# twndus/YelpRecommendation

Hardware: AMD Instinct MI355X
Metric: BPR triplets/sec @ dim64 (higher is better)
Workload: dtype f32; 1 GPU; BPR-MF dim=64 train step (gather+score+loss+grad+dense Adam), synthetic Yelp2018 shape; users=31668, items=38048, interactions=1566260, train_triplets_per_epoch=920629, batch_per_gpu=524288, global_batch=524288, optimizer=adam(dense), parallelism=single

## Files before the change

include/yelprec_engine.h:

```cpp
#ifndef YELPREC_ENGINE_H
#define YELPREC_ENGINE_H

#include <stdint.h>

#ifdef __cplusplus
extern "C" {
#endif

#define YR_ENGINE_VERSION 31

#define YR_ERR_UNSUPPORTED (-1)
#define YR_ERR_BADARG      (-2)

#define YR_FLAG_BAD_USER 1
#define YR_FLAG_BAD_ITEM 2

#define YR_PULL_USER_PHASE 1
#define YR_PULL_ITEM_PHASE 2

#define YR_OPT_ADAM  0
#define YR_OPT_ADAMW 1

#define YR_LOSS_PARTIALS 2048
#define YR_COUNT_SLOTS 64
#define YR_COUNT_WORDS 2048

int yr_engine_version(void);

const char *yr_engine_arch(void);

int yr_mf_score(const float *U, const float *I,
                const int64_t *user, const int64_t *item,
// ... 31 lines not shown
int yr_bpr_mf_pull_step(const float *U_old, float *U_new, float *I,
                        float *mU, float *vU, float *mI, float *vI, float *gradI_out,
                        const int64_t *user, const int64_t *pos, const int64_t *neg,
                        int64_t B, int D, int64_t num_users, int64_t num_items, float inv_batch,
                        double lr, double step_size, double bc2_sqrt,
                        double beta1, double beta2, double eps, double weight_decay, int mode,
                        int deterministic, void *workspace, int64_t workspace_bytes,
                        float *loss_partials, float *loss_out, double *loss_accum,
                        int32_t *err_flag, void *stream);

int yr_bpr_mf_pull_index(const int64_t *user, const int64_t *pos, const int64_t *neg, int64_t B, int D,
                         int64_t num_users, int64_t num_items,
                         void *workspace, int64_t workspace_bytes, int32_t *err_flag, void *stream);
int yr_bpr_mf_pull_apply(const float *U_old, float *U_new, float *I,
                         float *mU, float *vU, float *mI, float *vI, float *gradI_out,
                         int64_t B, int D, int64_t num_users, int64_t num_items, float inv_batch,
                         double lr, double step_size, double bc2_sqrt,
                         double beta1, double beta2, double eps, double weight_decay, int mode,
                         int deterministic, void *workspace, int64_t workspace_bytes,
                         float *loss_partials, float *loss_out, double *loss_accum,
                         int phases, int64_t item_row_begin, int64_t item_row_end,
                         void *stream);
int yr_bpr_mf_pull_item_buckets(int64_t num_items, int D);
int yr_bpr_mf_pull_apply_ordered(const float *U_old, float *U_new, float *I,
                         float *mU, float *vU, float *mI, float *vI, float *gradI_out,
                         int64_t B, int D, int64_t num_users, int64_t num_items, float inv_batch,
                         double lr, double step_size, double bc2_sqrt,
                         double beta1, double beta2, double eps, double weight_decay, int mode,
                         int deterministic, void *workspace, int64_t workspace_bytes,
                         float *loss_partials, float *loss_out, double *loss_accum,
                         int phases, int64_t item_row_begin, int64_t item_row_end,
                         const int32_t *item_bucket_order, void *stream);

#define YR_NGCF_MAX_LAYERS 8
int yr_ngcf_score_fwd(const float *const *layers, int n_layers, const int64_t *user, const int64_t *pos,
                      const int64_t *neg, int64_t B, int D, int64_t num_users, int64_t num_items,
                      float *out_pos, float *out_neg, int32_t *err_flag, void *stream);
int yr_ngcf_score_bwd(const float *const *layers, float *const *dlayers, int n_layers, const int64_t *user,
                      const int64_t *pos, const int64_t *neg, const float *gpos, const float *gneg,
                      int64_t B, int D, int64_t num_users, int64_t num_items, int32_t *err_flag, void *stream);
int yr_spmm_csr(const int32_t *rowptr, const int32_t *col, const float *val,
                const float *X, float *Y, int64_t n, int D, int accumulate,
                const int32_t *heavy_rows, int64_t n_heavy, int heavy_threshold, void *stream);
int yr_spmm_csr_sliced(const int32_t *rowptr, const int32_t *col, const float *val,
                       const float *X, float *Y, int64_t n, int D, int accumulate,
                       const int32_t *row_order, void *stream);
// ... 217 lines not shown
```

yelprecommendation_amd/_lib.py:

```python
from __future__ import annotations

import ctypes as C
import os

_HERE = os.path.dirname(os.path.abspath(__file__))
LIB_PATH = os.environ.get("YR_ENGINE_LIB") or os.path.join(_HERE, "libyelprec_engine.so")
ENGINE_VERSION = 31

_p = C.c_void_p
_i64 = C.c_int64
_int = C.c_int
_f = C.c_float
_d = C.c_double

SIGNATURES = {
    "yr_engine_version": [],
    "yr_engine_arch": [],
    "yr_mf_score": [_p, _p, _p, _p, _i64, _int, _i64, _i64, _p, _p, _p],
    "yr_mf_score_backward": [_p, _p, _p, _p, _p, _i64, _int, _i64, _i64, _p, _p, _p, _p],
    "yr_bpr_mf_fwd_bwd": [_p, _p, _p, _p, _p, _i64, _int, _i64, _i64, _f, _p, _p, _p, _p, _p],
    "yr_bpr_mf_scatter_step": [_p, _p, _p, _p, _p, _p, _p, _p, _p, _p, _p, _p, _i64, _int, _i64, _i64, _f,
                               _d, _d, _d, _d, _d, _d, _d, _int, _p, _p, _p, _p, _p],
    "yr_adam_dense_dual": [_p, _p, _p, _p, _i64, _p, _p, _p, _p, _i64, _int, _p, _p,
                           _d, _d, _d, _d, _d, _d, _d, _int, _p, _f, _p, _p, _p],
    "yr_bpr_mf_pull_workspace_bytes": [_i64, _i64, _i64, _int],
    "yr_bpr_mf_pull_step": [_p, _p, _p, _p, _p, _p, _p, _p, _p, _p, _p, _i64, _int, _i64, _i64, _f,
                            _d, _d, _d, _d, _d, _d, _d, _int, _int, _p, _i64, _p, _p, _p, _p, _p],
    "yr_spmm_csr": [_p, _p, _p, _p, _p, _i64, _int, _int, _p, _i64, _int, _p],
    "yr_spmm_csr_sliced": [_p, _p, _p, _p, _p, _i64, _int, _int, _p, _p],
    "yr_ngcf_score_fwd": [_p, _int, _p, _p, _p, _i64, _int, _i64, _i64, _p, _p, _p, _p],
# ... 20 lines not shown
    "yr_cdae_train_lists": [_p, _p, _p, _p, _p, _i64, _i64, _i64, _int, C.c_uint64, C.c_uint64, _d, _p, _p, _p, _p, _p,
                            _p, _p, _p],
    "yr_cdae_train_lists_batched": [_p, _p, _p, _p, _p, _i64, _i64, _i64, _int, _p, _p, _i64, _d, _p, _p, _p, _p, _p,
                                    _p, _p, _p],
    "yr_cdae_loss_finalize_batched": [_p, _int, _p, _i64, _i64, _p, _p, _p, _p],
    "yr_cdae_loss_finalize": [_p, _i64, _p, _p, _p, _p],
    "yr_cdae_sampled_decode_splits": [_i64],
    "yr_cdae_sampled_decode": [_p, _p, _p, _p, _p, _p, _i64, _i64, _int, _int, _p, _p, _p, _p, _p, _p],
    "yr_cdae_hidden_init": [_p, _p, _p, _p, _i64, _int, _i64, _p, _p],
    "yr_dropout": [_p, _p, _d, _i64, _p, _p],
    "yr_sigmoid": [_p, _i64, _p],
    "yr_dropout_seeded": [_p, C.c_uint64, _d, _i64, _p, _p],
    "yr_sigmoid_bwd": [_p, _p, _p, _i64, _p],
    "yr_colsum": [_p, _i64, _i64, _p, _int, _p],
    "yr_row_scatter_add": [_p, _p, _i64, _int, _i64, _p, _p],
    "yr_nsbce_fwd": [_p, _p, _p, _i64, _p, _p, _p],
    "yr_nsbce_bwd": [_p, _p, _p, _p, _p, _i64, _p, _p],
    "yr_bpr_mf_pull_index": [_p, _p, _p, _i64, _int, _i64, _i64, _p, _i64, _p, _p],
    "yr_bpr_mf_pull_apply": [_p, _p, _p, _p, _p, _p, _p, _p, _i64, _int, _i64, _i64, _f,
                             _d, _d, _d, _d, _d, _d, _d, _int, _int, _p, _i64, _p, _p, _p, _int, _i64, _i64, _p],
    "yr_bpr_mf_pull_apply_ordered": [_p, _p, _p, _p, _p, _p, _p, _p, _i64, _int, _i64, _i64, _f,
                             _d, _d, _d, _d, _d, _d, _d, _int, _int, _p, _i64, _p, _p, _p, _int, _i64, _i64, _p, _p],
    "yr_bpr_mf_pull_item_buckets": [_i64, _int],
    "yr_loss_finalize": [_p, _f, _p, _p, _p],
    "yr_mf_scores_gemm": [_p, _p, _p, _i64, _int, _i64, _i64, _p, _i64, _p, _p],
    "yr_mf_eval_topk_planes_bytes": [_i64, _int],
    "yr_mf_eval_topk_workspace_bytes": [_i64, _i64, _int, _int, _int],
    "yr_mf_eval_topk": [_p, _p, _p, _i64, _int, _i64, _i64, _p, _p, _f, _int, _p, _p, _i64, _int, _p, _p, _p],
    "yr_mf_eval_topk_bias": [_p, _p, _p, _p, _i64, _int, _i64, _i64, _p, _p, _f, _int, _p, _p, _i64, _int, _p, _p, _p],
    "yr_topk_masked": [_p, _i64, _i64, _i64, _p, _p, _p, _f, _int, _p, _p],
    "yr_rank_metrics_workspace_bytes": [_i64],
    "yr_rank_metrics": [_p, _i64, _int, _p, _p, _p, _p, _p, _p],
    "yr_bpr_loss_fwd": [_p, _p, _i64, _p, _p],
    "yr_bpr_loss_bwd": [_p, _p, _p, _f, _i64, _p, _p, _p],
    "yr_adam_dense": [_p, _p, _p, _p, _i64, _d, _d, _d, _d, _d, _d, _d, _int, _int, _p],
    "yr_adam_dense_flat": [_p, _p, _p, _p, _p, _p, _p, _p, _p, _p, _int, _d, _d, _d, _d, _d, _d, _d, _int, _p],
    "yr_csr_rows_to_dense": [_p, _p, _p, _i64, _i64, _i64, _int, _p, _p, _p],
    "yr_negative_mask": [_p, _i64, _i64, _int, C.c_uint64, _p, _p, _p],
    "yr_sgd_dense": [_p, _p, _i64, _d, _d, _int, _p],
    "yr_cdae_sparse_part_columns": [_i64],
    "yr_cdae_compact_rows": [_p, _i64, _i64, C.c_uint64, _d, _p, _p, _p, _p],
    "yr_cdae_sparse_encode": [_p, _p, _p, _p, _p, _p, _p, _i64, _i64, _int, _i64, _int, _p, _p, _p],
    "yr_cdae_sparse_dwh": [_p, _p, _p, _p, _i64, _i64, _int, _p, _p, _p, C.c_int32, _p, _p, _p],
    "yr_cdae_sparse_encode_t": [_p, _p, _p, _p, _p, _p, _p, _i64, _i64, _int, _i64, _int, _p, _p, _p],
    "yr_cdae_sparse_dwh_t": [_p, _p, _p, _p, _i64, _i64, _int, _p, _p, _p],
    "yr_cdae_hidden_bwd_dwh_t": [_p, _p, _p, _p, _p, _int, _int, _p, _p, _i64, _i64, _int, _i64, _p, _p, _p, _p, _p, _p,
# ... 67 lines not shown
```

yelprecommendation_amd/csrc/bpr_pull.hip:

```cpp
#include "adam.h"
#include "common.h"

namespace yr {

constexpr int kPartThreads = 1024;
#ifndef YR_ITEM_CAP
#define YR_ITEM_CAP 1024
#endif
constexpr int kCap = YR_ITEM_CAP;
constexpr int kUserCap = 768;
constexpr int kTileGroup = 256;
constexpr int kOccShift = 26;
constexpr int kOccMask = (1 << kOccShift) - 1;
constexpr int kMaxBuckets = 16383;
constexpr int kMaxOwnerGrid = 4096;
#ifndef YR_HEAVY_ROW
#define YR_HEAVY_ROW 96
#endif
constexpr int kHeavyRow = YR_HEAVY_ROW;
#ifndef YR_SPLIT_MIN
#define YR_SPLIT_MIN 2048
#endif
constexpr int kSplitMin = YR_SPLIT_MIN;
#ifndef YR_SPLIT_AVG_MIN
#define YR_SPLIT_AVG_MIN 2.5
#endif
#ifndef YR_SPLIT_AVG_TARGET
#define YR_SPLIT_AVG_TARGET 1.25
#endif
#ifndef YR_SPLIT_TARGET
#define YR_SPLIT_TARGET 1024
#endif
constexpr int kSplitTarget = YR_SPLIT_TARGET;
constexpr int kMaxParts = 64;
constexpr int kMaxTasks = 512;
constexpr int kMaxSlots = 1024;
constexpr int kBuildLanes = 4;
#ifndef YR_DEAL
#define YR_DEAL 1
#endif
#ifndef YR_DEAL_MIN
#define YR_DEAL_MIN 256
#endif
constexpr int kDealMin = YR_DEAL_MIN;
#ifndef YR_OWNER_WAVES
#define YR_OWNER_WAVES 8
#endif

struct PullAdam {
  AdamScalars c;
  int decoupled;
};

__device__ __forceinline__ float4 ld4o(const float* base, uint32_t off) {
  return *reinterpret_cast<const float4*>(reinterpret_cast<const char*>(base) + (uint32_t)(off * 4u));
}

template <int D>
struct PullGeom {
// ... 8 lines not shown
constexpr int kMinTiles = YR_MIN_TILES;
constexpr int kNarrowRows = kWavesPerBlock;
constexpr int kNarrowShift = 2;
#ifndef YR_NARROW_BELOW
#define YR_NARROW_BELOW 768
#endif
constexpr int kNarrowBelow = YR_NARROW_BELOW;

inline int bucket_shift(int D) { return D == 16 ? 6 : D == 32 ? 5 : D == 64 ? 4 : 3; }

template <int PT>
__global__ __launch_bounds__(kPartThreads) void tile_partition_kernel(
    const int64_t* __restrict__ user, const int64_t* __restrict__ pos, const int64_t* __restrict__ neg, int64_t B,
    int64_t nU, int64_t nI, int shiftU, int shiftI, int nbU, int nbI, int32_t* __restrict__ offU,
    int32_t* __restrict__ offI,
    int4* __restrict__ rec, int2* __restrict__ occ, int32_t* __restrict__ err_flag, int stage_off,
    int32_t* __restrict__ split_counters) {
  extern __shared__ int32_t s_cnt[];
  __shared__ int s_wave[kPartThreads / kWave];
  int4* s_stage = reinterpret_cast<int4*>(s_cnt + stage_off);
  constexpr int TILE = kPartThreads * PT;
  const int side = blockIdx.y, tile = blockIdx.x, tid = threadIdx.x;
  if (side == 0 && tile == 0) {
    if (tid < 2) split_counters[tid] = 0;
    for (int i = tid; i < nbI; i += kPartThreads) split_counters[4 + i] = 1;
  }
  const int nb = side ? nbI : nbU;
  const int shift = side ? shiftI : shiftU;
  const int rmask = (1 << shift) - 1;

  int32_t u[PT], p[PT], n[PT];
  int bad = 0;
#pragma unroll
  for (int k = 0; k < PT; ++k) {
    const int64_t b = (int64_t)tile * TILE + (int64_t)k * kPartThreads + tid;
    u[k] = -1; p[k] = 0; n[k] = 0;
    if (b < B) {
      const int64_t uu = user[b], pp = pos[b], nn = neg[b];
      int f = 0;
      if ((uint64_t)uu >= (uint64_t)nU) f |= YR_FLAG_BAD_USER;
      if ((uint64_t)pp >= (uint64_t)nI || (uint64_t)nn >= (uint64_t)nI) f |= YR_FLAG_BAD_ITEM;
      if (f) bad |= f;
      else { u[k] = (int32_t)uu; p[k] = (int32_t)pp; n[k] = (int32_t)nn; }
    }
  }
  for (int i = tid; i <= nb; i += kPartThreads) s_cnt[i] = 0;
  __syncthreads();
// ... 79 lines not shown
  const float* other;
  float* m;
  float* v;
  float* grad_out;
  const int32_t* off;
  const void* recs;
  float* coeff;
  float* loss_partials;
  float* loss_out;
  double* loss_accum;
  int finalize;
  int nb, T, tile_stride;
  int rows;
  int bucket_begin, bucket_end;
  const int32_t* order;
  int heavy_t;
  float inv_batch;
  PullAdam adam;
  char* split;
  float* scratch;
  const int32_t* b_off;
  int helper_blocks, build_blocks, b_nb;
  int b_split_min, b_split_target;
};

__host__ __device__ __forceinline__ size_t split_per(int nbI) { return ((size_t)nbI * 4 + 15) & ~(size_t)15; }
__device__ __forceinline__ int32_t* split_counters(char* b) { return (int32_t*)b; }
__device__ __forceinline__ int32_t* split_parts(char* b) { return (int32_t*)(b + 16); }
__device__ __forceinline__ int32_t* split_slot(char* b, int nbI) { return (int32_t*)(b + 16 + split_per(nbI)); }
__device__ __forceinline__ int32_t* split_arrive(char* b, int nbI) { return (int32_t*)(b + 16 + 2 * split_per(nbI)); }
__device__ __forceinline__ int4* split_tasks(char* b, int nbI) { return (int4*)(b + 16 + 3 * split_per(nbI)); }

__device__ __forceinline__ void build_splits(const OwnerArgs& a, int builder) {
  const int k = (builder * kBlock + (int)threadIdx.x) / kBuildLanes, j = threadIdx.x % kBuildLanes;
  int total = 0;
  if (k < a.b_nb) {
    int t = j;
    const int64_t pitch = a.b_nb + 1;
    for (; t + 3 * kBuildLanes < a.T; t += 4 * kBuildLanes) {
      const int32_t* o0 = a.b_off + (int64_t)t * pitch + k;
      const int32_t* o1 = o0 + kBuildLanes * pitch;
      const int32_t* o2 = o1 + kBuildLanes * pitch;
      const int32_t* o3 = o2 + kBuildLanes * pitch;
      const int a0 = o0[0], b0 = o0[1], a1 = o1[0], b1 = o1[1], a2 = o2[0], b2 = o2[1], a3 = o3[0], b3 = o3[1];
      total += ((b0 - a0) + (b1 - a1)) + ((b2 - a2) + (b3 - a3));
    }
    for (; t < a.T; t += kBuildLanes) {
      const int32_t* orow = a.b_off + (int64_t)t * (a.b_nb + 1) + k;
      total += orow[1] - orow[0];
    }
  }
#pragma unroll
  for (int m = 1; m < kBuildLanes; m <<= 1) total += __shfl_xor(total, m, kWave);
  if (k >= a.b_nb || j != 0) return;
  int parts = 1;
  if (total >= a.b_split_min) {
    parts = (total + a.b_split_target - 1) / a.b_split_target;
    parts = min(parts, min(kMaxParts, a.T));
  }
  int slot = 0;
  if (parts > 1) {
    slot = atomicAdd(split_counters(a.split) + 1, parts);
    const int first = atomicAdd(split_counters(a.split), parts - 1);
    const bool fits = slot + parts <= kMaxSlots && first + parts - 1 <= kMaxTasks;
    for (int q = 1; q < parts; ++q)
      if (first + q - 1 < kMaxTasks) split_tasks(a.split, a.b_nb)[first + q - 1] = make_int4(fits ? k : -1, q, 0, 0);
    if (!fits) parts = 1;
  }
  split_parts(a.split)[k] = parts;
  split_slot(a.split, a.b_nb)[k] = slot;
  split_arrive(a.split, a.b_nb)[k] = 0;
}

template <int LPR>
__device__ __forceinline__ void cross_group_sum(float4& a) {
#pragma unroll
  for (int m = LPR; m < kWave; m <<= 1) {
    a.x += __shfl_xor(a.x, m, kWave);
    a.y += __shfl_xor(a.y, m, kWave);
    a.z += __shfl_xor(a.z, m, kWave);
    a.w += __shfl_xor(a.w, m, kWave);
  }
}

__device__ __forceinline__ int wave_inclusive_scan(int x, int lane) {
#pragma unroll
  for (int d = 1; d < kWave; d <<= 1) {
    const int t = __shfl_up(x, d, kWave);
    if (lane >= d) x += t;
  }
  return x;
// ... 104 lines not shown
        part = fmaf(ownj.z, d.z, part);
        part = fmaf(ownj.w, d.w, part);
        const float x = group_sum_dpp<LPR>(part);
        float sp, sg;
        bpr_terms(x, sp, sg);
        const float gg = valid[q] ? -sg * a.inv_batch : 0.0f;
        cur.x = fmaf(gg, d.x, cur.x); cur.y = fmaf(gg, d.y, cur.y);
        cur.z = fmaf(gg, d.z, cur.z); cur.w = fmaf(gg, d.w, cur.w);
        if (valid[q] && l == 0) {
          a.coeff[ic[q]] = gg;
          loss += sp;
        }
      } else {
        const float gg = valid[q] ? __int_as_float(ib[q]) : 0.0f;
        cur.x = fmaf(gg, r0[q].x, cur.x); cur.y = fmaf(gg, r0[q].y, cur.y);
        cur.z = fmaf(gg, r0[q].z, cur.z); cur.w = fmaf(gg, r0[q].w, cur.w);
      }
    }
  }
  if (!HEAVY) {
    const int slot = LOOKUP ? (int)s_slotof[max(cur_row, 0)] : cur_row;
    sums.book(cur_row >= 0, slot - row_base, cur, grp);
  }
}

template <int D, bool USER, bool FUSE_ADAM, bool DET, int RPWX = 0>
__global__ __launch_bounds__(kBlock, YR_OWNER_WAVES) void owner_pass_kernel(OwnerArgs a) {
  using G = PullGeom<D>;
  constexpr int LPR = G::LPR, GPW = G::GPW;
  constexpr int RPW = RPWX ? RPWX : GPW;
  static_assert(RPW <= GPW, "a wave finishes at most one row per lane group");
  constexpr int R = kWavesPerBlock * RPW;
  constexpr int DEAL_BAR = kDealMin * (kWavesPerBlock * GPW) * (kWavesPerBlock * GPW) / 256;
  constexpr bool DEAL = RPWX == 0 && YR_DEAL && DEAL_BAR <= (USER ? kUserCap : kCap);
  constexpr bool TAG_SLOT = DEAL && !USER, LOOKUP = DEAL && USER;
  constexpr int CAP = USER ? kUserCap : kCap;
  constexpr int PT = CAP / kBlock;
  __shared__ int s_pre[kTileGroup + 1];
  __shared__ int s_base[kTileGroup];
  __shared__ int s_cnt[kWave];
  __shared__ int s_start[kWave];
  __shared__ int s_light[kWave + 1];
  __shared__ unsigned char s_slotof[DEAL ? kWave : 1];
  __shared__ unsigned char s_rowof[DEAL ? kWave : 1];
  __shared__ int s_x[CAP];
  __shared__ int s_y[CAP];
// ... 6 lines not shown
  __shared__ int s_n;
  const int tid = threadIdx.x, lane = tid & (kWave - 1), wave = tid / kWave;
  const int grp = lane / LPR, l = lane % LPR;
  const bool finisher = grp < RPW;
  const int row_l = wave * RPW + (finisher ? grp : 0);
  float loss = 0.0f;
  __shared__ int s_last;
  if (USER && (int)blockIdx.x < a.build_blocks) {
    build_splits(a, blockIdx.x);
    return;
  }
  const int hb = USER ? a.build_blocks : a.helper_blocks;
  const bool helper = !USER && (int)blockIdx.x < hb;
  const int owners = (int)gridDim.x - hb;
#ifdef YR_STAMPS
  bool first_bucket = true;
  int walk_iters = 0, heavy_iters = 0;
#endif
  YR_STAMP(0);

  for (int ks = helper ? (int)blockIdx.x : a.bucket_begin + (int)blockIdx.x - hb;
       helper ? ks == (int)blockIdx.x : ks < a.bucket_end; ks += owners) {
    int k, part = 0, parts = 1;
    const bool pools_hold = USER || !a.split || (split_counters(a.split)[0] <= kMaxTasks &&
                                                 split_counters(a.split)[1] <= kMaxSlots);
    if (helper) {
      if (!pools_hold || ks >= split_counters(a.split)[0]) break;
      const int4 task = split_tasks(a.split, a.nb)[ks];
      k = __builtin_amdgcn_readfirstlane(task.x);
      part = __builtin_amdgcn_readfirstlane(task.y);
      if (k < a.bucket_begin || k >= a.bucket_end) break;
    } else {
      k = __builtin_amdgcn_readfirstlane(a.order ? a.order[ks] : ks);
    }
    if (!USER && a.split && pools_hold) parts = __builtin_amdgcn_readfirstlane(split_parts(a.split)[k]);
    const int t_begin = __builtin_amdgcn_readfirstlane(a.T * part / parts);
    const int t_end = __builtin_amdgcn_readfirstlane(a.T * (part + 1) / parts);
    int row_t = row_l;
    int row_f = k * R + row_t;
    bool valid_f = finisher && row_f < a.rows;
    uint32_t o_f = (uint32_t)(row_f * D + 4 * l);
    bool bound = false;
    if (USER && finisher) s_own[row_l * LPR + l] = valid_f ? ld4o(a.own_old, o_f) : zero4();
    YR_STAMP(1);
    RowSums<LPR, GPW> sums;
    sums.clear();

    for (int tg0 = t_begin; tg0 < t_end; tg0 += kTileGroup) {
      const int nt = min(kTileGroup, t_end - tg0);
      int len = 0;
      if (tid < nt) {
        const int32_t* orow = a.off + (int64_t)(tg0 + tid) * (a.nb + 1) + k;
        const int o0 = orow[0], o1 = orow[1];
        len = o1 - o0;
        s_base[tid] = (tg0 + tid) * a.tile_stride + o0;
      }
      int inc = 0, before = 0;
      if (nt > kWave) {
        inc = wave_inclusive_scan(len, lane);
        if (lane == kWave - 1) s_scan[wave] = inc;
        __syncthreads();
        for (int w = 0; w < wave; ++w) before += s_scan[w];
      } else if (wave == 0) {
// ... 30 lines not shown
        }
        if (tid < kWave) s_cnt[tid] = 0;
        if (DET && tid == 0) s_n = 0;
        __syncthreads();
        int key[PT];
        int n_rec = cend - c0;
        if (DET && windowed) {
          constexpr int W = USER ? CAP : CAP / 2;
          const int tile_ids = USER ? a.tile_stride : a.tile_stride >> 1;
          const int seg = s_pre[wt + 1] - s_pre[wt];
          const uint32_t rbase = (uint32_t)s_base[wt];
          const uint32_t id_lo = (uint32_t)(tg0 + wt) * (uint32_t)tile_ids + (uint32_t)sub * (uint32_t)W;
          for (int sidx = tid; sidx < seg; sidx += kBlock) {
            if (USER) {
              const int4 r = static_cast<const int4*>(a.recs)[rbase + sidx];
              if ((uint32_t)r.z - id_lo < (uint32_t)W) {
                const int slot = atomicAdd(&s_n, 1);
                s_x[slot] = r.x; s_y[slot] = r.y; s_z[slot] = r.z;
                s_idx[slot] = (unsigned short)r.w;
              }
            } else {
              const int2 oc = static_cast<const int2*>(a.recs)[rbase + sidx];
              const uint32_t b = (uint32_t)(oc.y & 0x7fffffff);
              if (b - id_lo < (uint32_t)W) {
                const float g = a.coeff[b];
                const int slot = atomicAdd(&s_n, 1);
                s_x[slot] = oc.x & kOccMask;
                s_y[slot] = __float_as_int(oc.y < 0 ? -g : g);
                s_z[slot] = oc.y;
                s_idx[slot] = (unsigned short)((uint32_t)oc.x >> kOccShift);
              }
            }
          }
          __syncthreads();
          n_rec = s_n;
#pragma unroll
          for (int q = 0; q < PT; ++q) {
            const int c = tid + q * kBlock;
            key[q] = -1;
            if (c < n_rec) {
              const int local = s_idx[c];
              key[q] = local | (atomicAdd(&s_cnt[local], 1) << 8);
            }
          }
          ++sub;
          if (sub * W >= tile_ids) { sub = 0; cend = s_pre[wt + 1]; }
          else cend = c0;
// ... 13 lines not shown
            if (s_pre[mid] <= j) tlo = mid; else thi = mid;
          }
          addr[q] = j < cend ? (uint32_t)(s_base[tlo] + (j - s_pre[tlo])) : 0u;
        }
        if (USER) {
          int4 r[PT];
#pragma unroll
          for (int q = 0; q < PT; ++q)
            r[q] = *reinterpret_cast<const int4*>(static_cast<const char*>(a.recs) + (uint32_t)(addr[q] * 16u));
#pragma unroll
          for (int q = 0; q < PT; ++q)
            if (key[q] >= 0) {
              const int c = tid + q * kBlock;
              s_x[c] = r[q].x; s_y[c] = r[q].y; s_z[c] = r[q].z;
              key[q] = r[q].w | (atomicAdd(&s_cnt[r[q].w], 1) << 8);
            }
        } else {
          int2 oc[PT];
          float g[PT];
#pragma unroll
          for (int q = 0; q < PT; ++q)
            oc[q] = *reinterpret_cast<const int2*>(static_cast<const char*>(a.recs) + (uint32_t)(addr[q] * 8u));
#pragma unroll
          for (int q = 0; q < PT; ++q) {
            const uint32_t b = key[q] >= 0 ? (uint32_t)(oc[q].y & 0x7fffffff) : 0u;
            g[q] = *reinterpret_cast<const float*>(reinterpret_cast<const char*>(a.coeff) + (uint32_t)(b * 4u));
          }
#pragma unroll
          for (int q = 0; q < PT; ++q)
            if (key[q] >= 0) {
              const int c = tid + q * kBlock;
              const int local = (int)((uint32_t)oc[q].x >> kOccShift);
              s_x[c] = oc[q].x & kOccMask;
              s_y[c] = __float_as_int(oc[q].y < 0 ? -g[q] : g[q]);
              if (DET) s_z[c] = oc[q].y;
              key[q] = local | (atomicAdd(&s_cnt[local], 1) << 8);
            }
        }
        }
        __syncthreads();
        if (wave == 0) {
          if (DEAL && !bound) {
            if (n_rec >= DEAL_BAR) {
              deal_rows<R, RPW>(s_cnt, s_slotof, s_rowof, lane, a.heavy_t);
            } else {
              s_slotof[lane] = (unsigned char)lane;
              s_rowof[lane] = (unsigned char)lane;
            }
            __builtin_amdgcn_fence(__ATOMIC_ACQ_REL, "wavefront");
            __builtin_amdgcn_wave_barrier();
          }
          const int row = DEAL ? (int)s_rowof[lane] : lane;
          const int c = s_cnt[row];
          const bool heavy = c > a.heavy_t;
          const int cl = heavy ? 0 : c, ch = heavy ? c : 0;
          const int il = wave_inclusive_scan(cl, lane), ih = wave_inclusive_scan(ch, lane);
          const int total_light = __shfl(il, kWave - 1, kWave);
          s_light[lane] = il - cl;
          if (lane == kWave - 1) s_light[kWave] = il;
          s_start[row] = heavy ? total_light + ih - ch : il - cl;
        }
        bound = true;
        __syncthreads();
#pragma unroll
        for (int q = 0; q < PT; ++q)
          if (key[q] >= 0) {
            const int row = key[q] & 255;
            const int tag = TAG_SLOT ? (int)s_slotof[row] : row;
            s_idx[s_start[row] + (key[q] >> 8)] = (unsigned short)((tid + q * kBlock) | (tag << kTagShift));
          }
        __syncthreads();
        if (DET) {
          int at[PT];
          unsigned short ent[PT];
#pragma unroll
          for (int q = 0; q < PT; ++q) {
            const int pos = tid + q * kBlock;
            at[q] = -1;
            if (pos < n_rec) {
              ent[q] = s_idx[pos];
              const int r = TAG_SLOT ? (int)s_rowof[ent[q] >> kTagShift] : ent[q] >> kTagShift;
              const uint32_t mine = (uint32_t)s_z[ent[q] & ((1 << kTagShift) - 1)];
              const int lo = s_start[r], cnt = s_cnt[r];
              int before = 0;
              for (int j = lo; j < lo + cnt; ++j)
                before += (uint32_t)s_z[s_idx[j] & ((1 << kTagShift) - 1)] < mine ? 1 : 0;
// ... 28 lines not shown
#endif
            cross_group_sum<LPR>(t);
            if (grp == 0) s_heavy[wave][l] = t;
            __syncthreads();
            if (finisher && row_l == (DEAL ? (int)s_slotof[r] : r)) {
#pragma unroll
              for (int w = 0; w < kWavesPerBlock; ++w) {
                const float4 h = s_heavy[w][l];
                sums.total.x += h.x; sums.total.y += h.y; sums.total.z += h.z; sums.total.w += h.w;
              }
            }
            __syncthreads();
          }
        }
        __syncthreads();
      }
    }

    YR_STAMP(3);
    float4 acc = sums.finish(grp);
    if (DEAL) {
      if (bound) row_t = s_rowof[row_l];
      row_f = k * R + row_t;
      valid_f = row_f < a.rows;
      int t2 = tid;
      asm volatile("" : "+v"(t2));
      o_f = (uint32_t)(row_f * D + 4 * (t2 % LPR));
    }
    if (!USER && parts > 1) {
      float* sbase = a.scratch;
      asm volatile("" : "+s"(sbase));
      float* slots = sbase + (int64_t)split_slot(a.split, a.nb)[k] * (R * D);
      if (finisher) st4(slots + (int64_t)part * (R * D) + row_t * D + 4 * l, acc);
      __threadfence();
      __syncthreads();
      if (tid == 0) {
        s_last = atomicAdd(split_arrive(a.split, a.nb) + k, 1) == parts - 1;
        if (s_last) split_arrive(a.split, a.nb)[k] = 0;
      }
      __syncthreads();
      const bool last = s_last != 0;
      __syncthreads();
      if (!last) continue;
      __threadfence();
      acc = zero4();
      if (finisher) {
        for (int q = 0; q < parts; ++q) {
          const float4 t = ld4(slots + (int64_t)q * (R * D) + row_t * D + 4 * l);
          acc.x += t.x; acc.y += t.y; acc.z += t.z; acc.w += t.w;
        }
      }
    }
    if (valid_f) {
      if (FUSE_ADAM) {
        float4 own = USER ? s_own[row_t * LPR + l] : ld4o(a.own_old, o_f);
        float4 M = ld4o(a.m, o_f), V = ld4o(a.v, o_f);
        adam_element(own.x, acc.x, M.x, V.x, a.adam.c, a.adam.decoupled);
        adam_element(own.y, acc.y, M.y, V.y, a.adam.c, a.adam.decoupled);
        adam_element(own.z, acc.z, M.z, V.z, a.adam.c, a.adam.decoupled);
        adam_element(own.w, acc.w, M.w, V.w, a.adam.c, a.adam.decoupled);
        st4(a.own_new + o_f, own);
        st4(a.m + o_f, M);
        st4(a.v + o_f, V);
      } else {
        st4(a.grad_out + o_f, acc);
      }
    }
    YR_STAMP(4);
    if (USER) __syncthreads();
    YR_STAMP(5);
#ifdef YR_STAMPS
// ... 24 lines not shown
    }
  }
}

__global__ __launch_bounds__(kBlock) void pull_loss_finalize_kernel(const float* __restrict__ partials, float scale,
                                                                    float* __restrict__ loss_out,
                                                                    double* __restrict__ loss_accum) {
  __shared__ float s_red[kWavesPerBlock];
  float s = 0.0f;
  for (int i = threadIdx.x; i < YR_LOSS_PARTIALS; i += kBlock) s += partials[i];
  const float total = block_sum(s, s_red);
  if (threadIdx.x == 0) {
    const float v = total * scale;
    if (loss_out) loss_out[0] = v;
    if (loss_accum) loss_accum[0] += (double)v;
  }
}

inline size_t align16(size_t x) { return (x + 15) & ~(size_t)15; }
struct PullPlan {
  int pt, tile, T, shiftU, shiftI, narrow_users, nbU, nbI;
  size_t o_offU, o_offI, o_rec, o_occ, o_coeff, o_split, o_scratch, bytes;
};
inline size_t split_bytes(int nbI) { return 16 + (size_t)3 * align16((size_t)nbI * 4) + (size_t)kMaxTasks * sizeof(int4); }

inline int tile_pt(int64_t B) {
  int pt = 4;
  while (pt > 1 && (B + (int64_t)kPartThreads * pt - 1) / ((int64_t)kPartThreads * pt) < kMinTiles) pt >>= 1;
  return pt;
}

inline PullPlan make_plan(int64_t B, int64_t nU, int64_t nI, int D, bool upper_bound) {
  PullPlan p;
  p.shiftI = bucket_shift(D);
  const int R = 1 << p.shiftI;
  p.narrow_users = (nU + R - 1) / R < kNarrowBelow && R > kNarrowRows;
  p.shiftU = p.narrow_users ? kNarrowShift : p.shiftI;
  p.nbU = (int)((nU + (1 << p.shiftU) - 1) >> p.shiftU);
  p.nbI = (int)((nI + (1 << p.shiftI) - 1) >> p.shiftI);
  p.pt = tile_pt(B);
  p.tile = kPartThreads * p.pt;
  p.T = (int)((B + p.tile - 1) / p.tile);
  const int64_t T = upper_bound ? ((B + 4095) / 4096 > 2 * kMinTiles ? (B + 4095) / 4096 : 2 * kMinTiles) : p.T;
  const int64_t slots = upper_bound ? B + 4096 : (int64_t)p.T * p.tile;
  size_t o = 0;
  p.o_offU = o; o += align16((size_t)T * (p.nbU + 1) * 4);
  p.o_offI = o; o += align16((size_t)T * (p.nbI + 1) * 4);
  p.o_rec = o; o += align16((size_t)slots * sizeof(int4));
  p.o_occ = o; o += align16((size_t)slots * 2 * sizeof(int2));
  p.o_coeff = o; o += align16((size_t)(B > 0 ? B : 1) * 4);
  p.o_split = o; o += align16(split_bytes(p.nbI));
  p.o_scratch = o; o += (size_t)kMaxSlots * 1024 * 4;
  p.bytes = o;
  return p;
}

}

using namespace yr;

static int pull_check_common(int64_t B, int D, int64_t num_users, int64_t num_items, const void* workspace,
                             int64_t workspace_bytes) {
  if (B < 0 || num_users <= 0 || num_items <= 0 || B > 0x3fffffff) return YR_ERR_BADARG;
  if (D != 16 && D != 32 && D != 64 && D != 128) return YR_ERR_UNSUPPORTED;
  const PullPlan pl = make_plan(0, num_users, num_items, D, false);
  if (pl.nbU > kMaxBuckets || pl.nbI > kMaxBuckets) return YR_ERR_UNSUPPORTED;
  if (num_users > kOccMask) return YR_ERR_UNSUPPORTED;
  if (!workspace || (reinterpret_cast<uintptr_t>(workspace) & 15u) != 0) return YR_ERR_BADARG;
  if ((int64_t)make_plan(B, num_users, num_items, D, false).bytes > workspace_bytes) return YR_ERR_BADARG;
  return 0;
}

#ifdef YR_STAMPS
extern "C" int yr_debug_read_stamps(long long* host, int n) {
  return (int)hipMemcpyFromSymbol(host, HIP_SYMBOL(g_stamps), sizeof(long long) * n);
}
extern "C" int yr_debug_read_walk_iters(int* host, int n) {
// ... 47 lines not shown
  return launch_status();
}

template <int D>
static int pull_apply_impl(const float* U_old, float* U_new, float* I, float* mU, float* vU, float* mI, float* vI,
                           float* gradI_out, int64_t B, int64_t nU, int64_t nI, float inv_batch, const PullAdam& adam,
                           int deterministic, void* workspace, float* loss_partials, float* loss_out,
                           double* loss_accum, int phases, int64_t item_begin, int64_t item_end,
                           const int32_t* item_order, hipStream_t s) {
  const PullPlan p = make_plan(B, nU, nI, D, false);
  char* w = static_cast<char*>(workspace);
  const bool want_loss = loss_out || loss_accum;
  if (phases & YR_PULL_USER_PHASE) {
    OwnerArgs ua{};
    ua.own_old = U_old; ua.own_new = U_new; ua.other = I; ua.m = mU; ua.v = vU; ua.grad_out = nullptr;
    ua.off = (const int32_t*)(w + p.o_offU); ua.recs = w + p.o_rec; ua.coeff = (float*)(w + p.o_coeff);
    ua.loss_partials = loss_partials;
    ua.nb = p.nbU; ua.T = p.T; ua.tile_stride = p.tile; ua.rows = (int)nU;
    ua.bucket_begin = 0; ua.bucket_end = p.nbU;
    ua.order = nullptr;
    ua.heavy_t = kHeavyRow; ua.inv_batch = inv_batch; ua.adam = adam;
    ua.build_blocks = (p.nbI * kBuildLanes + kBlock - 1) / kBlock;
    ua.b_off = (const int32_t*)(w + p.o_offI); ua.b_nb = p.nbI;
    {
      const double avg = 2.0 * (double)B / (double)p.nbI;
      const int by_avg_min = (int)(YR_SPLIT_AVG_MIN * avg), by_avg_target = (int)(YR_SPLIT_AVG_TARGET * avg);
      ua.b_split_min = by_avg_min > kSplitMin ? by_avg_min : kSplitMin;
      ua.b_split_target = by_avg_target > kSplitTarget ? by_avg_target : kSplitTarget;
    }
    ua.split = w + p.o_split;
    const int gu = (p.nbU < YR_LOSS_PARTIALS ? p.nbU : YR_LOSS_PARTIALS) + ua.build_blocks;
    if (p.narrow_users && deterministic)
      hipLaunchKernelGGL((owner_pass_kernel<D, true, true, true, 1>), dim3(gu), dim3(kBlock), 0, s, ua);
    else if (p.narrow_users)
      hipLaunchKernelGGL((owner_pass_kernel<D, true, true, false, 1>), dim3(gu), dim3(kBlock), 0, s, ua);
    else if (deterministic)
      hipLaunchKernelGGL((owner_pass_kernel<D, true, true, true>), dim3(gu), dim3(kBlock), 0, s, ua);
    else
      hipLaunchKernelGGL((owner_pass_kernel<D, true, true, false>), dim3(gu), dim3(kBlock), 0, s, ua);
  }
  const bool items = (phases & YR_PULL_ITEM_PHASE) && item_end > item_begin;
  if (items) {
    OwnerArgs ia{};
    ia.own_old = I; ia.own_new = I; ia.other = U_old; ia.m = mI; ia.v = vI; ia.grad_out = gradI_out;
    ia.off = (const int32_t*)(w + p.o_offI); ia.recs = w + p.o_occ; ia.coeff = (float*)(w + p.o_coeff);
    ia.loss_partials = loss_partials; ia.loss_out = loss_out; ia.loss_accum = loss_accum;
    ia.finalize = want_loss ? 1 : 0;
    ia.nb = p.nbI; ia.T = p.T; ia.tile_stride = 2 * p.tile; ia.rows = (int)nI;
    ia.bucket_begin = (int)(item_begin >> p.shiftI);
    ia.bucket_end = (int)((item_end + (1 << p.shiftI) - 1) >> p.shiftI);
    ia.order = (item_order && ia.bucket_begin == 0 && ia.bucket_end == p.nbI) ? item_order : nullptr;
    ia.heavy_t = kHeavyRow; ia.inv_batch = inv_batch; ia.adam = adam;
    ia.helper_blocks = kMaxTasks;
    ia.split = w + p.o_split;
    ia.scratch = (float*)(w + p.o_scratch);
    int gi = ia.bucket_end - ia.bucket_begin;
    if (gi > kMaxOwnerGrid) gi = kMaxOwnerGrid;
    gi += kMaxTasks;
    if (gradI_out && deterministic)
      hipLaunchKernelGGL((owner_pass_kernel<D, false, false, true>), dim3(gi), dim3(kBlock), 0, s, ia);
    else if (gradI_out)
      hipLaunchKernelGGL((owner_pass_kernel<D, false, false, false>), dim3(gi), dim3(kBlock), 0, s, ia);
    else if (deterministic)
      hipLaunchKernelGGL((owner_pass_kernel<D, false, true, true>), dim3(gi), dim3(kBlock), 0, s, ia);
    else
      hipLaunchKernelGGL((owner_pass_kernel<D, false, true, false>), dim3(gi), dim3(kBlock), 0, s, ia);
  } else if (want_loss) {
    hipLaunchKernelGGL(pull_loss_finalize_kernel, dim3(1), dim3(kBlock), 0, s, loss_partials, inv_batch, loss_out,
                       loss_accum);
  }
  return launch_status();
}

extern "C" int yr_bpr_mf_pull_item_buckets(int64_t num_items, int D) {
  if (num_items <= 0 || (D != 16 && D != 32 && D != 64 && D != 128)) return YR_ERR_BADARG;
  const int sh = bucket_shift(D);
  return (int)((num_items + (1 << sh) - 1) >> sh);
}

extern "C" int yr_bpr_mf_pull_apply_ordered(const float* U_old, float* U_new, float* I, float* mU, float* vU,
                                            float* mI, float* vI, float* gradI_out, int64_t B, int D,
                                            int64_t num_users, int64_t num_items, float inv_batch, double lr,
                                            double step_size, double bc2_sqrt, double beta1, double beta2, double eps,
                                            double weight_decay, int mode, int deterministic, void* workspace,
                                            int64_t workspace_bytes, float* loss_partials, float* loss_out,
                                            double* loss_accum, int phases, int64_t item_row_begin,
                                            int64_t item_row_end, const int32_t* item_bucket_order, void* stream) {
  int rc = pull_check_common(B, D, num_users, num_items, workspace, workspace_bytes);
  if (rc) return rc;
  if (!(phases & (YR_PULL_USER_PHASE | YR_PULL_ITEM_PHASE))) return YR_ERR_BADARG;
  if (item_row_begin < 0 || item_row_end > num_items || item_row_begin > item_row_end) return YR_ERR_BADARG;
  const int R = 1 << bucket_shift(D);
  if (item_row_begin % R != 0 || (item_row_end % R != 0 && item_row_end != num_items)) return YR_ERR_BADARG;
  if (!U_old || !U_new || U_old == U_new || !I || !mU || !vU || !loss_partials) return YR_ERR_BADARG;
  if (!gradI_out && (!mI || !vI)) return YR_ERR_BADARG;
  if (mode != YR_OPT_ADAM && mode != YR_OPT_ADAMW) return YR_ERR_UNSUPPORTED;
  const PullAdam c = {adam_scalars(lr, step_size, bc2_sqrt, beta1, beta2, eps, weight_decay), mode == YR_OPT_ADAMW};
  hipStream_t s = (hipStream_t)stream;
#define YR_APPLY_CASE(DD)                                                                                       \
  case DD:                                                                                                      \
// ... 45 lines not shown
```

yelprecommendation_amd/engine.py:

```python
from __future__ import annotations

import torch

from . import _lib
from ._lib import EngineError, check

LOSS_PARTIALS = 2048
FLAG_BAD_USER, FLAG_BAD_ITEM = 1, 2
OPT_ADAM, OPT_ADAMW = 0, 1
PULL_USER_PHASE, PULL_ITEM_PHASE = 1, 2
SUPPORTED_WIDTHS = (16, 32, 64, 128)
WIDE_WIDTHS = (256, 512, 1024)
MF_WIDTHS = SUPPORTED_WIDTHS + WIDE_WIDTHS


_raw_stream = getattr(torch._C, "_cuda_getCurrentRawStream", None)


def _stream() -> int:
    if _raw_stream is not None:
        return _raw_stream(torch.cuda.current_device())
    return torch.cuda.current_stream().cuda_stream


# ... 87 lines not shown
PULL_MAX_BUCKETS = 16383
PULL_MAX_USERS = (1 << 26) - 1


def pull_bucket_rows(d):
    return 1024 // int(d)


def pull_supported(num_users, num_items, d):
    if d not in SUPPORTED_WIDTHS:
        return False
    r = pull_bucket_rows(d)
    ru = 4 if (-(-num_users // r) < 768 and r > 4) else r
    return (-(-num_users // ru) <= PULL_MAX_BUCKETS and -(-num_items // r) <= PULL_MAX_BUCKETS
            and num_users <= PULL_MAX_USERS)


def bpr_mf_pull_workspace(max_batch, num_users, num_items, d, device):
    lib = _lib.load()
    n = lib.yr_bpr_mf_pull_workspace_bytes(int(max_batch), int(num_users), int(num_items), int(d))
    if n < 0:
        check(int(n), "yr_bpr_mf_pull_workspace_bytes")
    return torch.empty(int(n), dtype=torch.uint8, device=device)


def bpr_mf_pull_step(U_old, U_new, I, mU, vU, mI, vI, user, pos, neg, step, lr, loss_partials, workspace,
                     beta1=0.9, beta2=0.999, eps=1e-8, weight_decay=0.0, decoupled=False, inv_batch=None,
                     gradI_out=None, err_flag=None, loss_out=None, loss_accum=None, deterministic=False):
    lib = _lib.load()
    nu, ni, d = _table_dims(U_old, I)
    B = user.numel()
    if pos.numel() != B or neg.numel() != B:
        raise EngineError("user/pos/neg index tensors differ in length")
    if U_new.shape != U_old.shape or U_new.data_ptr() == U_old.data_ptr():
        raise EngineError("U_new must be a distinct buffer of U_old's shape")
    if loss_partials.numel() != LOSS_PARTIALS:
        raise EngineError(f"loss_partials must hold {LOSS_PARTIALS} floats")
    if inv_batch is None:
        inv_batch = 1.0 / B if B else 0.0
    step_size, bc2_sqrt = adam_scalars(step, lr, beta1, beta2)
    f32 = torch.float32
    check(lib.yr_bpr_mf_pull_step(
        _dev(U_old, f32, "U_old"), _dev(U_new, f32, "U_new"), _dev(I, f32, "I"),
        _dev(mU, f32, "mU"), _dev(vU, f32, "vU"), _opt(mI, f32, "mI"), _opt(vI, f32, "vI"),
        _opt(gradI_out, f32, "gradI_out"),
        _dev(user, torch.int64, "user"), _dev(pos, torch.int64, "pos"), _dev(neg, torch.int64, "neg"),
# ... 973 lines not shown
```

Before: 4.758 billion triplets/s.

## Split moderately heavy item buckets across helper blocks by row interleaving

Adds a second load-balancing mode for item buckets: buckets that are heavy but below the existing temporal-split threshold are divided into 2 or 4 parts by row residue. Each helper block processes only the rows whose index matches its part, so no scratch reduction is needed. Row tasks are queued from the top of the helper task pool, and a summary API is added for inspecting the split decisions. The aim is to cut tail latency from skewed item buckets. The cost is extra filtering work on every record in split buckets, because each block still scans the bucket's full record list.

```diff
diff --git a/include/yelprec_engine.h b/include/yelprec_engine.h
--- a/include/yelprec_engine.h
+++ b/include/yelprec_engine.h
@@ -7,7 +7,7 @@
 extern "C" {
 #endif
 
-#define YR_ENGINE_VERSION 31
+#define YR_ENGINE_VERSION 32
 
 #define YR_ERR_UNSUPPORTED (-1)
 #define YR_ERR_BADARG      (-2)
@@ -85,6 +85,9 @@
                          int phases, int64_t item_row_begin, int64_t item_row_end,
                          void *stream);
 int yr_bpr_mf_pull_item_buckets(int64_t num_items, int D);
+int yr_bpr_mf_pull_split_summary(const void *workspace, int64_t workspace_bytes, int64_t B, int D,
+                                 int64_t num_users, int64_t num_items, int32_t *counters_out,
+                                 int32_t *parts_out, int32_t *rule_out, void *stream);
 int yr_bpr_mf_pull_apply_ordered(const float *U_old, float *U_new, float *I,
                          float *mU, float *vU, float *mI, float *vI, float *gradI_out,
                          int64_t B, int D, int64_t num_users, int64_t num_items, float inv_batch,
diff --git a/yelprecommendation_amd/_lib.py b/yelprecommendation_amd/_lib.py
--- a/yelprecommendation_amd/_lib.py
+++ b/yelprecommendation_amd/_lib.py
@@ -5,7 +5,7 @@
 
 _HERE = os.path.dirname(os.path.abspath(__file__))
 LIB_PATH = os.environ.get("YR_ENGINE_LIB") or os.path.join(_HERE, "libyelprec_engine.so")
-ENGINE_VERSION = 31
+ENGINE_VERSION = 32
 
 _p = C.c_void_p
 _i64 = C.c_int64
@@ -72,6 +72,7 @@
     "yr_bpr_mf_pull_apply_ordered": [_p, _p, _p, _p, _p, _p, _p, _p, _i64, _int, _i64, _i64, _f,
                              _d, _d, _d, _d, _d, _d, _d, _int, _int, _p, _i64, _p, _p, _p, _int, _i64, _i64, _p, _p],
     "yr_bpr_mf_pull_item_buckets": [_i64, _int],
+    "yr_bpr_mf_pull_split_summary": [_p, _i64, _i64, _int, _i64, _i64, _p, _p, _p, _p],
     "yr_loss_finalize": [_p, _f, _p, _p, _p],
     "yr_mf_scores_gemm": [_p, _p, _p, _i64, _int, _i64, _i64, _p, _i64, _p, _p],
     "yr_mf_eval_topk_planes_bytes": [_i64, _int],
diff --git a/yelprecommendation_amd/csrc/bpr_pull.hip b/yelprecommendation_amd/csrc/bpr_pull.hip
--- a/yelprecommendation_amd/csrc/bpr_pull.hip
+++ b/yelprecommendation_amd/csrc/bpr_pull.hip
@@ -35,6 +35,24 @@
 constexpr int kMaxParts = 64;
 constexpr int kMaxTasks = 512;
 constexpr int kMaxSlots = 1024;
+#ifndef YR_ROWSPLIT
+#define YR_ROWSPLIT 1
+#endif
+#ifndef YR_ROWSPLIT_MIN
+#define YR_ROWSPLIT_MIN 1024
+#endif
+#ifndef YR_ROWSPLIT_AVG_MIN
+#define YR_ROWSPLIT_AVG_MIN 2.32
+#endif
+#ifndef YR_ROWSPLIT_TARGET
+#define YR_ROWSPLIT_TARGET 512
+#endif
+#ifndef YR_ROWSPLIT_AVG_TARGET
+#define YR_ROWSPLIT_AVG_TARGET 1.16
+#endif
+constexpr int kRowSplitMin = YR_ROWSPLIT_MIN;
+constexpr int kRowSplitTarget = YR_ROWSPLIT_TARGET;
+constexpr int kMaxRowTasks = YR_ROWSPLIT ? 512 : 0;
 constexpr int kBuildLanes = 4;
 #ifndef YR_DEAL
 #define YR_DEAL 1
@@ -89,7 +107,7 @@
   constexpr int TILE = kPartThreads * PT;
   const int side = blockIdx.y, tile = blockIdx.x, tid = threadIdx.x;
   if (side == 0 && tile == 0) {
-    if (tid < 2) split_counters[tid] = 0;
+    if (tid < 3) split_counters[tid] = 0;
     for (int i = tid; i < nbI; i += kPartThreads) split_counters[4 + i] = 1;
   }
   const int nb = side ? nbI : nbU;
@@ -215,6 +233,7 @@
   const int32_t* b_off;
   int helper_blocks, build_blocks, b_nb;
   int b_split_min, b_split_target;
+  int b_rowsplit_min, b_rowsplit_quad;
 };
 
 __host__ __device__ __forceinline__ size_t split_per(int nbI) { return ((size_t)nbI * 4 + 15) & ~(size_t)15; }
@@ -223,6 +242,7 @@
 __device__ __forceinline__ int32_t* split_slot(char* b, int nbI) { return (int32_t*)(b + 16 + split_per(nbI)); }
 __device__ __forceinline__ int32_t* split_arrive(char* b, int nbI) { return (int32_t*)(b + 16 + 2 * split_per(nbI)); }
 __device__ __forceinline__ int4* split_tasks(char* b, int nbI) { return (int4*)(b + 16 + 3 * split_per(nbI)); }
+__device__ __forceinline__ int2* split_row_tasks(char* b, int nbI) { return (int2*)(split_tasks(b, nbI) + kMaxTasks); }
 
 __device__ __forceinline__ void build_splits(const OwnerArgs& a, int builder) {
   const int k = (builder * kBlock + (int)threadIdx.x) / kBuildLanes, j = threadIdx.x % kBuildLanes;
@@ -260,6 +280,15 @@
       if (first + q - 1 < kMaxTasks) split_tasks(a.split, a.b_nb)[first + q - 1] = make_int4(fits ? k : -1, q, 0, 0);
     if (!fits) parts = 1;
   }
+#if YR_ROWSPLIT
+  else if (total < a.b_split_min && total >= a.b_rowsplit_min) {
+    const int S = total >= a.b_rowsplit_quad ? 4 : 2;
+    const int first = atomicAdd(split_counters(a.split) + 2, S - 1);
+    for (int q = 1; q < S; ++q)
+      if (first + q - 1 < kMaxRowTasks) split_row_tasks(a.split, a.b_nb)[first + q - 1] = make_int2(k, q);
+    parts = -S;
+  }
+#endif
   split_parts(a.split)[k] = parts;
   split_slot(a.split, a.b_nb)[k] = slot;
   split_arrive(a.split, a.b_nb)[k] = 0;
@@ -410,6 +439,10 @@
     const int slot = LOOKUP ? (int)s_slotof[max(cur_row, 0)] : cur_row;
     sums.book(cur_row >= 0, slot - row_base, cur, grp);
   }
+}
+
+__device__ __forceinline__ bool row_kept(int row, int part, int parts) {
+  return !YR_ROWSPLIT || ((row ^ part) & max(-parts - 1, 0)) == 0;
 }
 
 template <int D, bool USER, bool FUSE_ADAM, bool DET, int RPWX = 0>
@@ -462,23 +495,43 @@
   for (int ks = helper ? (int)blockIdx.x : a.bucket_begin + (int)blockIdx.x - hb;
        helper ? ks == (int)blockIdx.x : ks < a.bucket_end; ks += owners) {
     int k, part = 0, parts = 1;
-    const bool pools_hold = USER || !a.split || (split_counters(a.split)[0] <= kMaxTasks &&
-                                                 split_counters(a.split)[1] <= kMaxSlots);
-    if (helper) {
-      if (!pools_hold || ks >= split_counters(a.split)[0]) break;
+    int4 cnt = make_int4(0, 0, 0, 0);
+    if (!USER && a.split) cnt = *reinterpret_cast<const int4*>(a.split);
+    int k_own = ks;
+    if (!helper && a.order) k_own = a.order[ks];
+    const int c_tasks = __builtin_amdgcn_readfirstlane(cnt.x), c_slots = __builtin_amdgcn_readfirstlane(cnt.y);
+    const int c_rows = __builtin_amdgcn_readfirstlane(cnt.z);
+    const bool pools_hold = USER || !a.split || (c_tasks <= kMaxTasks && c_slots <= kMaxSlots);
+    const int tile_tasks = (USER || !a.split || !pools_hold) ? 0 : c_tasks;
+    const bool rows_hold = !USER && YR_ROWSPLIT && a.split && c_rows <= kMaxRowTasks && tile_tasks + c_rows <= kMaxTasks;
+    const bool row_helper = YR_ROWSPLIT && helper && ks >= tile_tasks;
+    if (row_helper) {
+      const int j = kMaxTasks - 1 - ks;
+      if (!rows_hold || j >= c_rows) break;
+      const int2 task = split_row_tasks(a.split, a.nb)[j];
+      k = __builtin_amdgcn_readfirstlane(task.x);
+      part = __builtin_amdgcn_readfirstlane(task.y);
+      if (k < a.bucket_begin || k >= a.bucket_end) break;
+    } else if (helper) {
+      if (ks >= tile_tasks) break;
       const int4 task = split_tasks(a.split, a.nb)[ks];
       k = __builtin_amdgcn_readfirstlane(task.x);
       part = __builtin_amdgcn_readfirstlane(task.y);
       if (k < a.bucket_begin || k >= a.bucket_end) break;
     } else {
-      k = __builtin_amdgcn_readfirstlane(a.order ? a.order[ks] : ks);
-    }
-    if (!USER && a.split && pools_hold) parts = __builtin_amdgcn_readfirstlane(split_parts(a.split)[k]);
-    const int t_begin = __builtin_amdgcn_readfirstlane(a.T * part / parts);
-    const int t_end = __builtin_amdgcn_readfirstlane(a.T * (part + 1) / parts);
+      k = __builtin_amdgcn_readfirstlane(k_own);
+    }
+    if (!USER && a.split) {
+      const int word = __builtin_amdgcn_readfirstlane(split_parts(a.split)[k]);
+      if (word > 1 && pools_hold) parts = word;
+      if (YR_ROWSPLIT && word < 0 && rows_hold) parts = word;
+    }
+    if (row_helper && parts >= 0) break;
+    const int t_begin = parts < 0 ? 0 : __builtin_amdgcn_readfirstlane(a.T * part / parts);
+    const int t_end = parts < 0 ? a.T : __builtin_amdgcn_readfirstlane(a.T * (part + 1) / parts);
     int row_t = row_l;
     int row_f = k * R + row_t;
-    bool valid_f = finisher && row_f < a.rows;
+    bool valid_f = finisher && row_f < a.rows && (USER || row_kept(row_t, part, parts));
     uint32_t o_f = (uint32_t)(row_f * D + 4 * l);
     bool bound = false;
     if (USER && finisher) s_own[row_l * LPR + l] = valid_f ? ld4o(a.own_old, o_f) : zero4();
@@ -555,7 +608,7 @@
             } else {
               const int2 oc = static_cast<const int2*>(a.recs)[rbase + sidx];
               const uint32_t b = (uint32_t)(oc.y & 0x7fffffff);
-              if (b - id_lo < (uint32_t)W) {
+              if (b - id_lo < (uint32_t)W && row_kept((int)((uint32_t)oc.x >> kOccShift), part, parts)) {
                 const float g = a.coeff[b];
                 const int slot = atomicAdd(&s_n, 1);
                 s_x[slot] = oc.x & kOccMask;
@@ -615,6 +668,9 @@
           for (int q = 0; q < PT; ++q)
             oc[q] = *reinterpret_cast<const int2*>(static_cast<const char*>(a.recs) + (uint32_t)(addr[q] * 8u));
 #pragma unroll
+          for (int q = 0; q < PT; ++q)
+            if (!row_kept((int)((uint32_t)oc[q].x >> kOccShift), part, parts)) key[q] = -1;
+#pragma unroll
           for (int q = 0; q < PT; ++q) {
             const uint32_t b = key[q] >= 0 ? (uint32_t)(oc[q].y & 0x7fffffff) : 0u;
             g[q] = *reinterpret_cast<const float*>(reinterpret_cast<const char*>(a.coeff) + (uint32_t)(b * 4u));
@@ -634,7 +690,13 @@
         __syncthreads();
         if (wave == 0) {
           if (DEAL && !bound) {
-            if (n_rec >= DEAL_BAR) {
+            int n_deal = n_rec;
+            if (!USER && YR_ROWSPLIT && parts < 0) {
+              n_deal = s_cnt[lane];
+#pragma unroll
+              for (int m = 1; m < kWave; m <<= 1) n_deal += __shfl_xor(n_deal, m, kWave);
+            }
+            if (n_deal >= DEAL_BAR) {
               deal_rows<R, RPW>(s_cnt, s_slotof, s_rowof, lane, a.heavy_t);
             } else {
               s_slotof[lane] = (unsigned char)lane;
@@ -651,10 +713,12 @@
           const int total_light = __shfl(il, kWave - 1, kWave);
           s_light[lane] = il - cl;
           if (lane == kWave - 1) s_light[kWave] = il;
+          if (!USER && YR_ROWSPLIT && lane == kWave - 1) s_n = il + ih;
           s_start[row] = heavy ? total_light + ih - ch : il - cl;
         }
         bound = true;
         __syncthreads();
+        if (!USER && YR_ROWSPLIT && parts < 0) n_rec = __builtin_amdgcn_readfirstlane(s_n);
 #pragma unroll
         for (int q = 0; q < PT; ++q)
           if (key[q] >= 0) {
@@ -729,7 +793,7 @@
     if (DEAL) {
       if (bound) row_t = s_rowof[row_l];
       row_f = k * R + row_t;
-      valid_f = row_f < a.rows;
+      valid_f = row_f < a.rows && (USER || row_kept(row_t, part, parts));
       int t2 = tid;
       asm volatile("" : "+v"(t2));
       o_f = (uint32_t)(row_f * D + 4 * (t2 % LPR));
@@ -738,7 +802,10 @@
       float* sbase = a.scratch;
       asm volatile("" : "+s"(sbase));
       float* slots = sbase + (int64_t)split_slot(a.split, a.nb)[k] * (R * D);
-      if (finisher) st4(slots + (int64_t)part * (R * D) + row_t * D + 4 * l, acc);
+      int t3 = tid;
+      asm volatile("" : "+v"(t3));
+      const int lc = 4 * (t3 % LPR);
+      if (finisher) st4(slots + (int64_t)part * (R * D) + row_t * D + lc, acc);
       __threadfence();
       __syncthreads();
       if (tid == 0) {
@@ -753,7 +820,7 @@
       acc = zero4();
       if (finisher) {
         for (int q = 0; q < parts; ++q) {
-          const float4 t = ld4(slots + (int64_t)q * (R * D) + row_t * D + 4 * l);
+          const float4 t = ld4(slots + (int64_t)q * (R * D) + row_t * D + lc);
           acc.x += t.x; acc.y += t.y; acc.z += t.z; acc.w += t.w;
         }
       }
@@ -824,7 +891,9 @@
   int pt, tile, T, shiftU, shiftI, narrow_users, nbU, nbI;
   size_t o_offU, o_offI, o_rec, o_occ, o_coeff, o_split, o_scratch, bytes;
 };
-inline size_t split_bytes(int nbI) { return 16 + (size_t)3 * align16((size_t)nbI * 4) + (size_t)kMaxTasks * sizeof(int4); }
+inline size_t split_bytes(int nbI) {
+  return 16 + (size_t)3 * align16((size_t)nbI * 4) + (size_t)kMaxTasks * sizeof(int4) + (size_t)kMaxRowTasks * sizeof(int2);
+}
 
 inline int tile_pt(int64_t B) {
   int pt = 4;
@@ -855,6 +924,24 @@
   p.o_scratch = o; o += (size_t)kMaxSlots * 1024 * 4;
   p.bytes = o;
   return p;
+}
+
+struct SplitRule {
+  int split_min, split_target, row_min, row_target, row_quad, row_max_parts;
+};
+inline SplitRule split_rule(int64_t B, int nbI, int D) {
+  SplitRule r;
+  const double avg = 2.0 * (double)B / (double)nbI;
+  const int by_avg_min = (int)(YR_SPLIT_AVG_MIN * avg), by_avg_target = (int)(YR_SPLIT_AVG_TARGET * avg);
+  r.split_min = by_avg_min > kSplitMin ? by_avg_min : kSplitMin;
+  r.split_target = by_avg_target > kSplitTarget ? by_avg_target : kSplitTarget;
+  const int row_avg_min = (int)(YR_ROWSPLIT_AVG_MIN * avg), row_avg_target = (int)(YR_ROWSPLIT_AVG_TARGET * avg);
+  r.row_min = row_avg_min > kRowSplitMin ? row_avg_min : kRowSplitMin;
+  r.row_target = row_avg_target > kRowSplitTarget ? row_avg_target : kRowSplitTarget;
+  r.row_max_parts = D == 128 ? 2 : 4;
+  r.row_quad = r.row_max_parts >= 4 && r.row_target < 0x7fffffff / 3 ? 3 * r.row_target : 0x7fffffff;
+  if (!YR_ROWSPLIT) { r.row_min = 0x7fffffff; r.row_quad = 0x7fffffff; r.row_max_parts = 1; }
+  return r;
 }
 
 }
@@ -948,12 +1035,9 @@
     ua.heavy_t = kHeavyRow; ua.inv_batch = inv_batch; ua.adam = adam;
     ua.build_blocks = (p.nbI * kBuildLanes + kBlock - 1) / kBlock;
     ua.b_off = (const int32_t*)(w + p.o_offI); ua.b_nb = p.nbI;
-    {
-      const double avg = 2.0 * (double)B / (double)p.nbI;
-      const int by_avg_min = (int)(YR_SPLIT_AVG_MIN * avg), by_avg_target = (int)(YR_SPLIT_AVG_TARGET * avg);
-      ua.b_split_min = by_avg_min > kSplitMin ? by_avg_min : kSplitMin;
-      ua.b_split_target = by_avg_target > kSplitTarget ? by_avg_target : kSplitTarget;
-    }
+    const SplitRule rule = split_rule(B, p.nbI, D);
+    ua.b_split_min = rule.split_min; ua.b_split_target = rule.split_target;
+    ua.b_rowsplit_min = rule.row_min; ua.b_rowsplit_quad = rule.row_quad;
     ua.split = w + p.o_split;
     const int gu = (p.nbU < YR_LOSS_PARTIALS ? p.nbU : YR_LOSS_PARTIALS) + ua.build_blocks;
     if (p.narrow_users && deterministic)
@@ -982,7 +1066,7 @@
     ia.scratch = (float*)(w + p.o_scratch);
     int gi = ia.bucket_end - ia.bucket_begin;
     if (gi > kMaxOwnerGrid) gi = kMaxOwnerGrid;
-    gi += kMaxTasks;
+    gi += ia.helper_blocks;
     if (gradI_out && deterministic)
       hipLaunchKernelGGL((owner_pass_kernel<D, false, false, true>), dim3(gi), dim3(kBlock), 0, s, ia);
     else if (gradI_out)
@@ -1002,6 +1086,29 @@
   if (num_items <= 0 || (D != 16 && D != 32 && D != 64 && D != 128)) return YR_ERR_BADARG;
   const int sh = bucket_shift(D);
   return (int)((num_items + (1 << sh) - 1) >> sh);
+}
+
+extern "C" int yr_bpr_mf_pull_split_summary(const void* workspace, int64_t workspace_bytes, int64_t B, int D,
+                                            int64_t num_users, int64_t num_items, int32_t* counters_out,
+                                            int32_t* parts_out, int32_t* rule_out, void* stream) {
+  if (!rule_out || B <= 0 || num_users <= 0 || num_items <= 0) return YR_ERR_BADARG;
+  if (D != 16 && D != 32 && D != 64 && D != 128) return YR_ERR_UNSUPPORTED;
+  const PullPlan p = make_plan(B, num_users, num_items, D, false);
+  const SplitRule r = split_rule(B, p.nbI, D);
+  const int32_t rule[8] = {r.split_min, r.split_target, r.row_min, r.row_target, r.row_quad, r.row_max_parts,
+                           kMaxRowTasks, YR_ROWSPLIT};
+  for (int i = 0; i < 8; ++i) rule_out[i] = rule[i];
+  if (!workspace) return (counters_out || parts_out) ? YR_ERR_BADARG : 0;
+  const int rc = pull_check_common(B, D, num_users, num_items, workspace, workspace_bytes);
+  if (rc) return rc;
+  const char* blk = static_cast<const char*>(workspace) + p.o_split;
+  hipStream_t s = (hipStream_t)stream;
+  hipError_t e = hipSuccess;
+  if (counters_out) e = hipMemcpyAsync(counters_out, blk, 16, hipMemcpyDeviceToHost, s);
+  if (e == hipSuccess && parts_out)
+    e = hipMemcpyAsync(parts_out, blk + 16, (size_t)p.nbI * 4, hipMemcpyDeviceToHost, s);
+  if (e == hipSuccess) e = hipStreamSynchronize(s);
+  return (int)e;
 }
 
 extern "C" int yr_bpr_mf_pull_apply_ordered(const float* U_old, float* U_new, float* I, float* mU, float* vU,
diff --git a/yelprecommendation_amd/engine.py b/yelprecommendation_amd/engine.py
--- a/yelprecommendation_amd/engine.py
+++ b/yelprecommendation_amd/engine.py
@@ -133,6 +133,34 @@
     if n < 0:
         check(int(n), "yr_bpr_mf_pull_workspace_bytes")
     return torch.empty(int(n), dtype=torch.uint8, device=device)
+
+
+PULL_RULE_FIELDS = ("split_min", "split_target", "row_min", "row_target", "row_quad", "row_max_parts",
+                    "row_task_pool", "row_split_compiled")
+
+
+def bpr_mf_pull_split_summary(batch, num_users, num_items, d, workspace=None):
+    import ctypes
+    import numpy as np
+    lib = _lib.load()
+    rule = (ctypes.c_int32 * 8)()
+    counters = (ctypes.c_int32 * 4)()
+    nb = int(lib.yr_bpr_mf_pull_item_buckets(int(num_items), int(d)))
+    if nb < 0:
+        check(nb, "yr_bpr_mf_pull_item_buckets")
+    parts = np.zeros(nb, np.int32)
+    if workspace is None:
+        rc = lib.yr_bpr_mf_pull_split_summary(None, 0, int(batch), int(d), int(num_users), int(num_items), None, None,
+                                              rule, None)
+    else:
+        rc = lib.yr_bpr_mf_pull_split_summary(workspace.data_ptr(), workspace.numel(), int(batch), int(d),
+                                              int(num_users), int(num_items), counters, parts.ctypes.data, rule,
+                                              _stream())
+    check(rc, "yr_bpr_mf_pull_split_summary")
+    out = dict(zip(PULL_RULE_FIELDS, (int(v) for v in rule)))
+    if workspace is not None:
+        out.update(tasks=int(counters[0]), slots=int(counters[1]), row_tasks=int(counters[2]), parts=parts)
+    return out
 
 
 def bpr_mf_pull_step(U_old, U_new, I, mU, vU, mI, vI, user, pos, neg, step, lr, loss_partials, workspace,
```

Result: faster. 5.045 billion triplets/s, median of 6 (+6.0%).
